# levje/TrackToLearn

Measured on AMD Instinct MI355X. Metric: streamline-steps/s at n_actor=262144, higher is better.
Workload: dtype f32

## Files before the change

### tracktolearn_amd/csrc/ttl_hip.hip

```cpp
#include <hip/hip_runtime.h>

#include <atomic>
#include <chrono>
#include <cmath>
#include <cstdarg>
#include <cstdio>
#include <cstdlib>
#include <cstring>
#include <new>

#include "ttl_hip.h"

#include "ttl_internal.h"

#include <map>
#include <mutex>

namespace {
thread_local char g_err[512] = "";
}

int ttl_detail_fail(int code, const char *fmt, ...) {
    va_list ap;
    va_start(ap, fmt);
// ... 125 lines not shown
    float p1z, float p2x, float p2y, float p2z, int n_pts, float &ux, float &uy,
    float &uz, float &wx, float &wy, float &wz) {
    int bits = 0;
    if (n_pts >= P.max_nb_steps) bits |= TTL_FLAG_LENGTH;
    unit3(p2x - p1x, p2y - p1y, p2z - p1z, ux, uy, uz);
    wx = wy = wz = 0.f;
    if (n_pts >= 3) {
        unit3(p1x - p0x, p1y - p0y, p1z - p0z, wx, wy, wz);
        if (P.curv_enabled) {
            const float dot = (ux * wx + uy * wy) + uz * wz;
            if (dot <= P.curv_dot_max && dot >= -1.0f) bits |= TTL_FLAG_CURVATURE;
        }
    }
    if (outside_mask(P, p2x, p2y, p2z)) bits |= TTL_FLAG_MASK;
    return bits;
}

__device__ __forceinline__ void block_ranks(int *__restrict__ rank_out,
                                            int *__restrict__ counts_out, int i,
                                            bool active, bool keep) {
    const unsigned long long m = __ballot(keep);
    const int lane = threadIdx.x & 63;
    const int wave = threadIdx.x >> 6;
    const int below = __popcll(m & ((1ull << lane) - 1ull));
    __shared__ int wave_total[BLOCK / 64];
    if (lane == 0) wave_total[wave] = __popcll(m);
    __syncthreads();
    int before = 0;
#pragma unroll
    for (int w = 0; w < BLOCK / 64; ++w)
        if (w < wave) before += wave_total[w];
    if (active) rank_out[i] = before + below;
    if (threadIdx.x == 0) {
        int tot = 0;
#pragma unroll
        for (int w = 0; w < BLOCK / 64; ++w) tot += wave_total[w];
        counts_out[blockIdx.x] = tot;
    }
}

__device__ __forceinline__ void block_survivor_ranks(const EnvParams &P, int i,
                                                     bool active, bool keep) {
    block_ranks(P.rank, P.block_counts, i, active, keep);
}

template <int MODE>
__device__ __forceinline__ bool advance_row(
    const EnvParams &P, int g, int i, const float *__restrict__ actions,
    const double *__restrict__ noise, int L, double *__restrict__ reward_out,
    uint8_t *__restrict__ done_out) {
    bool stop = false;
    {
        float *h = P.hist + (size_t)g * (size_t)(P.max_nb_steps + 1) * 3;
        float4 *l2 = reinterpret_cast<float4 *>(P.last2 + 8 * (size_t)g);
        const float4 q0 = l2[0], q1 = l2[1];
        const float p0x = q0.x, p0y = q0.y, p0z = q0.z;
        const float p1x = q1.x, p1y = q1.y, p1z = q1.z;
        const float ax = actions[(size_t)i * 3 + 0];
        const float ay = actions[(size_t)i * 3 + 1];
        const float az = actions[(size_t)i * 3 + 2];

        float p2x, p2y, p2z;
        if (MODE == TTL_MODE_F32) {
            const float s = sqrtf((ax * ax + ay * ay) + az * az);
            float dx = (ax / s) * P.step32;
            float dy = (ay / s) * P.step32;
            float dz = (az / s) * P.step32;
            if (L == 1) {
                const float tx = p1x + dx, ty = p1y + dy, tz = p1z + dz;
                const bool flip = first_step_flips(P, tx, ty, tz);
                dx = flip ? -dx : dx;
                dy = flip ? -dy : dy;
                dz = flip ? -dz : dz;
            }
            p2x = p1x + dx;
            p2y = p1y + dy;
            p2z = p1z + dz;
        } else {
            double dx, dy, dz;
            if (MODE == TTL_MODE_F32NORM) {
                const float s = sqrtf((ax * ax + ay * ay) + az * az);
                dx = (double)(ax / s) * P.step64;
                dy = (double)(ay / s) * P.step64;
                dz = (double)(az / s) * P.step64;
            } else {
                double a0 = (double)ax, a1 = (double)ay, a2 = (double)az;
                if (noise) {
                    a0 = a0 + noise[(size_t)i * 3 + 0];
                    a1 = a1 + noise[(size_t)i * 3 + 1];
                    a2 = a2 + noise[(size_t)i * 3 + 2];
                } else {
                    a0 = a0 + 0.0;
                    a1 = a1 + 0.0;
                    a2 = a2 + 0.0;
                }
                const double s = sqrt((a0 * a0 + a1 * a1) + a2 * a2);
                dx = (a0 / s) * P.step64;
                dy = (a1 / s) * P.step64;
                dz = (a2 / s) * P.step64;
            }
            if (L == 1) {
                const float tx = (float)((double)p1x + dx);
                const float ty = (float)((double)p1y + dy);
                const float tz = (float)((double)p1z + dz);
                const bool flip = first_step_flips(P, tx, ty, tz);
                dx = flip ? -dx : dx;
                dy = flip ? -dy : dy;
                dz = flip ? -dz : dz;
            }
            p2x = (float)((double)p1x + dx);
            p2y = (float)((double)p1y + dy);
            p2z = (float)((double)p1z + dz);
        }
        h[L * 3 + 0] = p2x;
        h[L * 3 + 1] = p2y;
        h[L * 3 + 2] = p2z;
        l2[0] = q1;
        l2[1] = float4{p2x, p2y, p2z, 0.0f};

        const int n_pts = L + 1;
        float ux, uy, uz, wx, wy, wz;
        const int bits = stopping_bits(P, p0x, p0y, p0z, p1x, p1y, p1z, p2x, p2y,
                                       p2z, n_pts, ux, uy, uz, wx, wy, wz);

        stop = bits != 0;
        if (stop) {
            P.flags[g] = bits;
            P.dones[g] = 1;
        }
        done_out[i] = stop ? 1 : 0;

        if (reward_out) {
            double rew = 0.0;
            if (P.compute_reward && P.align_w > 0.0f) {
                int vi = (int)p1x, vj = (int)p1y, vk = (int)p1z;
                vi = min(max(vi, 0), P.peaks_dim[0] - 1);
                vj = min(max(vj, 0), P.peaks_dim[1] - 1);
                vk = min(max(vk, 0), P.peaks_dim[2] - 1);
                const float *pk =
                    P.peaks +
                    (((size_t)vi * P.peaks_dim[1] + vj) * P.peaks_dim[2] + vk) * 15;
                const float u0 = nan_to_num(ux), u1 = nan_to_num(uy),
                            u2 = nan_to_num(uz);
                float best = 0.f;
#pragma unroll
                for (int k = 0; k < 5; ++k) {
                    float vx, vy, vz;
                    unit3(pk[3 * k], pk[3 * k + 1], pk[3 * k + 2], vx, vy, vz);
                    vx = nan_to_num(vx);
                    vy = nan_to_num(vy);
                    vz = nan_to_num(vz);
                    const float d = fabsf((vx * u0 + vy * u1) + vz * u2);
                    if (k == 0)
                        best = d;
                    else if (best == best && (d != d || d > best))
                        best = d;
                }
                float r32 = best;
                if (n_pts >= 3) {
                    const double f = ((double)u0 * (double)nan_to_num(wx) +
                                      (double)u1 * (double)nan_to_num(wy)) +
                                     (double)u2 * (double)nan_to_num(wz);
                    r32 = (float)((double)r32 * f);
                }
                rew = (double)(P.align_w * r32);
            }
            reward_out[i] = rew;
        }
        P.stop[i] = stop ? 1 : 0;
        *reinterpret_cast<float4 *>(P.head + 4 * (size_t)i) =
            float4{p2x, p2y, p2z, __int_as_float(g)};
// ... 387 lines not shown
    if (n_pts >= 2) {
        bits = stopping_bits(P, t[0], t[1], t[2], t[3], t[4], t[5], t[6], t[7],
                             t[8], n_pts, ux, uy, uz, wx, wy, wz);
    } else {
        bits = (n_pts >= P.max_nb_steps) ? TTL_FLAG_LENGTH : 0;
        if (outside_mask(P, t[6], t[7], t[8])) bits |= TTL_FLAG_MASK;
    }
    out[i] = (uint8_t)bits;
}

__global__ __launch_bounds__(BLOCK) void k_finish(EnvParams P,
                                                  const int *__restrict__ idx,
                                                  int n_active, int n_pts) {
    const int i = blockIdx.x * BLOCK + threadIdx.x;
    if (i >= n_active) return;
    if (P.stop[i]) P.lengths[idx[i]] = n_pts;
}

__global__ __launch_bounds__(BLOCK) void k_copy_rows(
    EnvParams P, int n_active, int width, const float *__restrict__ in,
    float *__restrict__ out, long long pitch) {
    constexpr int LPS = 64;
    const int row = blockIdx.x * (BLOCK / LPS) + threadIdx.x / LPS;
    const int sub = threadIdx.x % LPS;
    if (row >= n_active) return;
    const int pos = P.surv_pos[row];
    if (pos < 0) return;
    const float *src = in + (size_t)row * (size_t)pitch;
    float *dst = out + (size_t)pos * (size_t)pitch;
    for (int f = sub; f < width; f += LPS) dst[f] = src[f];
}

__global__ __launch_bounds__(BLOCK) void k_pack_streamlines(
    const float *__restrict__ hist, long long row_pitch, const long long *__restrict__ keep,
    const long long *__restrict__ offsets, int n, float *__restrict__ out) {
    const int i = blockIdx.x * (BLOCK / 64) + (threadIdx.x >> 6);
    if (i >= n) return;
    const int lane = threadIdx.x & 63;
    const int floats = (int)keep[i] * 3;
    const float *src = hist + (size_t)i * (size_t)row_pitch;
    float *dst = out + (size_t)offsets[i] * 3;
    for (int f = lane; f < floats; f += 64) dst[f] = src[f];
}

__global__ __launch_bounds__(BLOCK) void k_reset(EnvParams P, int *idx,
                                                 const float *__restrict__ seeds,
                                                 int n) {
    const int i = blockIdx.x * BLOCK + threadIdx.x;
    if (i >= n) return;
    float *h = P.hist + (size_t)i * (size_t)(P.max_nb_steps + 1) * 3;
    h[0] = seeds[(size_t)i * 3 + 0];
    h[1] = seeds[(size_t)i * 3 + 1];
    h[2] = seeds[(size_t)i * 3 + 2];
    float4 *l2 = reinterpret_cast<float4 *>(P.last2 + 8 * (size_t)i);
    l2[0] = float4{0.0f, 0.0f, 0.0f, 0.0f};
    l2[1] = float4{h[0], h[1], h[2], 0.0f};
    P.flags[i] = 0;
    P.lengths[i] = 1;
    P.dones[i] = 0;
    idx[i] = i;
}

__global__ __launch_bounds__(BLOCK) void k_pack_sh(const float *__restrict__ src,
                                                   float *__restrict__ dst, int X, int Y,
                                                   int Z, int C, int pitch, int brick,
                                                   unsigned sx, unsigned sy) {
    const long long t = (long long)blockIdx.x * BLOCK + threadIdx.x;
    const long long total = (long long)X * Y * Z * pitch;
    if (t >= total) return;
    const long long v = t / pitch;
    const int c = (int)(t - v * pitch);
    const int z = (int)(v % Z), y = (int)((v / Z) % Y), x = (int)(v / ((long long)Z * Y));
    size_t rec;
    if (brick)
        rec = (size_t)(x >> 2) * sx + (size_t)(x & 3) * 16 + (size_t)(y >> 2) * sy +
              (size_t)(y & 3) * 4 + (size_t)(z >> 2) * 64 + (size_t)(z & 3);
    else
        rec = (size_t)v;
    dst[rec * pitch + c] = (c < C) ? src[v * C + c] : 0.0f;
}

__device__ __forceinline__ unsigned mix32(unsigned h) {
    h ^= h >> 16;
    h *= 0x85EBCA6Bu;
    h ^= h >> 13;
    h *= 0xC2B2AE35u;
    h ^= h >> 16;
    return h;
}

__device__ __forceinline__ float scripted_noise(unsigned seed, unsigned step,
                                                unsigned gid, unsigned comp) {
    const unsigned base = mix32(seed * 0x9E3779B1u + step) ^
                          mix32(gid * 0x27D4EB2Fu + comp * 0x165667B1u + 0x1234567u);
    float acc = 0.0f;
#pragma unroll
    for (unsigned k = 0; k < 4; ++k) {
        const unsigned h = mix32(base + k * 0x9E3779B9u);
        acc = acc + (float)(h >> 8) * 5.9604644775390625e-08f;
    }
    return (acc - 2.0f) * 1.7320508075688772f;
}

__global__ __launch_bounds__(BLOCK) void k_scripted_actions(
    const float *__restrict__ state, long long pitch, int dir_offset,
    const int *__restrict__ idx, int n, unsigned seed, unsigned step,
    float wobble, float *__restrict__ actions) {
    const int i = blockIdx.x * BLOCK + threadIdx.x;
    if (i >= n) return;
    const unsigned gid = (unsigned)idx[i];
    const float n0 = scripted_noise(seed, step, gid, 0);
    const float n1 = scripted_noise(seed, step, gid, 1);
    const float n2 = scripted_noise(seed, step, gid, 2);
    float a0 = n0, a1 = n1, a2 = n2;
    if (step > 0) {
        const float *row = state + (size_t)i * (size_t)pitch + dir_offset;
        const float px = row[0], py = row[1], pz = row[2];
        float s = sqrtf((px * px + py * py) + pz * pz);
        if (!(s > 0.0f)) s = 1.0f;
        a0 = px / s + wobble * n0;
        a1 = py / s + wobble * n1;
        a2 = pz / s + wobble * n2;
    }
    actions[(size_t)i * 3 + 0] = a0;
    actions[(size_t)i * 3 + 1] = a1;
    actions[(size_t)i * 3 + 2] = a2;
}

__global__ __launch_bounds__(BLOCK) void k_scripted_actions_fr(
    EnvParams P, const float *__restrict__ state, long long pitch, int dir_offset,
    const int *__restrict__ idx_a, const int *__restrict__ idx_b, int n_rows,
    unsigned seed, float wobble, float *__restrict__ actions) {
    const int *live = P.counts + TTL_FR_LIVE;
    const int n = min(live[0], n_rows);
    const unsigned step = (unsigned)(live[1] - 1);
    const int *idx = live[2] ? idx_b : idx_a;
    const int i = blockIdx.x * BLOCK + threadIdx.x;
    if (i >= n) return;
    const unsigned gid = (unsigned)idx[i];
    const float n0 = scripted_noise(seed, step, gid, 0);
    const float n1 = scripted_noise(seed, step, gid, 1);
    const float n2 = scripted_noise(seed, step, gid, 2);
    float a0 = n0, a1 = n1, a2 = n2;
    if (step > 0) {
        const float *row = state + (size_t)i * (size_t)pitch + dir_offset;
        const float px = row[0], py = row[1], pz = row[2];
        float s = sqrtf((px * px + py * py) + pz * pz);
        if (!(s > 0.0f)) s = 1.0f;
        a0 = px / s + wobble * n0;
        a1 = py / s + wobble * n1;
        a2 = pz / s + wobble * n2;
    }
    actions[(size_t)i * 3 + 0] = a0;
    actions[(size_t)i * 3 + 1] = a1;
    actions[(size_t)i * 3 + 2] = a2;
}

__global__ __launch_bounds__(BLOCK) void k_mask_classes(
    const double *__restrict__ coef, int nx, int ny, int nz, double thr,
    uint8_t *__restrict__ cls) {
    const long long t = (long long)blockIdx.x * BLOCK + threadIdx.x;
    const long long total = (long long)nx * ny * nz;
    if (t >= total) return;
    const int fz = (int)(t % nz), fy = (int)((t / nz) % ny), fx = (int)(t / ((long long)nz * ny));
    double lo = INFINITY, hi = -INFINITY;
    for (int a = 0; a < 4; ++a) {
        const int ia = mirror_fold(fx - 1 + a, nx);
        for (int b = 0; b < 4; ++b) {
            const int ib = mirror_fold(fy - 1 + b, ny);
            const double *line = coef + ((size_t)ia * ny + ib) * nz;
            for (int d = 0; d < 4; ++d) {
                const double v = line[mirror_fold(fz - 1 + d, nz)];
                lo = fmin(lo, v);
                hi = fmax(hi, v);
            }
        }
    }
    const double margin = 1e-9 * (1.0 + fabs(thr) + fmax(fabs(lo), fabs(hi)));
    uint8_t c = 0;
    if (lo >= thr + margin) c = 1;
    else if (hi < thr - margin) c = 2;
    if (!(lo == lo) || !(hi == hi)) c = 0;
    cls[t] = c;
}

inline size_t align_up(size_t v, size_t a) { return (v + a - 1) / a * a; }

}

struct ttl_env {
    ttl_env_desc d;
    EnvParams P;
    int length;
    int n_active;
    int cur;
    int stepped;
    int last_order;
    int last_n;
    uint8_t *last_done;
    int *proc[2];
    char *order_ws;
    size_t order_ws_bytes;
    int proc_cur;
    int use_proc;
    int n_slots;
    int tail_fused;
    int tail_fused_max;
    int state_kernel;
    hipStream_t side;
    hipEvent_t ev_prefix;
    hipEvent_t ev_counts;
    int counts_pending;
    const int32_t *host_counts;
    const int32_t *host_probe;
    int *host_dev;
    int poll_seq;
    hipStream_t poll_stream;
    int fuse_small;
    int poll_counts;
    int local_sort;
    int n_exact;
    int fr_cap;
    int *fr_host_word;
    int prof_on;
    int prof_mask;
    int prof_cap;
    int prof_n[TTL_PROFILE_CLASSES];
    hipEvent_t *prof_ev[TTL_PROFILE_CLASSES];
};

static void log_gather_rows(int n_rows) {
    static FILE *f = []() -> FILE * {
        const char *path = getenv("TTL_GATHER_ROWS_LOG");
        return path && *path ? fopen(path, "a") : nullptr;
    }();
    if (f) {
        fprintf(f, "%d\n", n_rows);
        fflush(f);
    }
}

static void prof_mark(ttl_env *e, int which, int stop, hipStream_t s) {
    if (!e->prof_on || !((e->prof_mask >> which) & 1) ||
        e->prof_n[which] >= e->prof_cap)
        return;
    (void)hipEventRecord(e->prof_ev[which][2 * e->prof_n[which] + stop], s);
    if (stop) e->prof_n[which]++;
}

extern "C" {

const char *ttl_last_error(void) { return g_err; }
uint32_t ttl_abi_version(void) { return TTL_ABI_VERSION; }
size_t ttl_env_desc_size(void) { return sizeof(ttl_env_desc); }

size_t ttl_env_workspace_bytes(int32_t n_max) {
    if (n_max < 0) return 0;
    const size_t n = (size_t)n_max;
    const size_t nb = (n + BLOCK - 1) / BLOCK + 1;
    size_t b = 0;
    b += align_up(n, 256);
    b += 6 * align_up(n * sizeof(int), 256);
    b += 2 * align_up(n * 4 * sizeof(float), 256);
    b += align_up(n * 8 * sizeof(float), 256);
    b += 2 * align_up(n * 2 * sizeof(int), 256);
    b += align_up(n * sizeof(int), 256);
    b += 2 * align_up(nb * sizeof(int), 256);
    b += 256;
    b += ttl_detail_order_workspace_bytes(n);
    return b;
}

int64_t ttl_sh_volume_records(const int32_t *dim, int32_t layout) {
    if (!dim || dim[0] < 1 || dim[1] < 1 || dim[2] < 1) return 0;
    if (layout == TTL_SH_BRICK4)
        return (int64_t)((dim[0] + 3) / 4) * ((dim[1] + 3) / 4) * ((dim[2] + 3) / 4) * 64;
    return (int64_t)dim[0] * dim[1] * dim[2];
}

struct VmmBlock {
    hipMemGenericAllocationHandle_t handle;
    size_t size;
};
static std::mutex g_vmm_mutex;
static std::map<void *, VmmBlock> g_vmm_blocks;

static hipError_t vmm_alloc(int device, size_t bytes, void **out) {
    hipMemAllocationProp prop{};
    prop.type = hipMemAllocationTypePinned;
    prop.location.type = hipMemLocationTypeDevice;
    prop.location.id = device;
    size_t gran = 0;
    hipError_t e = hipMemGetAllocationGranularity(&gran, &prop,
                                                  hipMemAllocationGranularityRecommended);
    if (e != hipSuccess || gran == 0) return e != hipSuccess ? e : hipErrorInvalidValue;
    const size_t size = (bytes + gran - 1) / gran * gran;
    VmmBlock b{};
    b.size = size;
    if ((e = hipMemCreate(&b.handle, size, &prop, 0)) != hipSuccess) return e;
    void *va = nullptr;
    if ((e = hipMemAddressReserve(&va, size, gran, nullptr, 0)) != hipSuccess) {
        (void)hipMemRelease(b.handle);
        return e;
    }
    hipMemAccessDesc acc{};
    acc.location = prop.location;
    acc.flags = hipMemAccessFlagsProtReadWrite;
    if ((e = hipMemMap(va, size, 0, b.handle, 0)) != hipSuccess ||
        (e = hipMemSetAccess(va, size, &acc, 1)) != hipSuccess) {
        (void)hipMemUnmap(va, size);
        (void)hipMemAddressFree(va, size);
        (void)hipMemRelease(b.handle);
        return e;
    }
    std::lock_guard<std::mutex> lock(g_vmm_mutex);
    g_vmm_blocks[va] = b;
    *out = va;
// ... 37 lines not shown

int ttl_volume_free(void *ptr) {
    if (!ptr) return TTL_OK;
    {
        std::unique_lock<std::mutex> lock(g_vmm_mutex);
        auto it = g_vmm_blocks.find(ptr);
        if (it != g_vmm_blocks.end()) {
            const VmmBlock b = it->second;
            g_vmm_blocks.erase(it);
            lock.unlock();
            HIP_TRY(hipDeviceSynchronize());
            HIP_TRY(hipMemUnmap(ptr, b.size));
            HIP_TRY(hipMemAddressFree(ptr, b.size));
            HIP_TRY(hipMemRelease(b.handle));
            return TTL_OK;
        }
    }
    HIP_TRY(hipFree(ptr));
    return TTL_OK;
}

int ttl_pack_sh_volume(const float *src, float *dst, const int32_t *dim, int32_t n_coef,
                       int32_t coef_pitch, int32_t layout, void *hip_stream) {
    if (!src || !dst || !dim || dim[0] < 1 || dim[1] < 1 || dim[2] < 1 || n_coef <= 0 ||
        coef_pitch < n_coef || (coef_pitch & 3) ||
        (layout != TTL_SH_LINEAR && layout != TTL_SH_BRICK4))
        return fail(TTL_ERR_INVALID, "ttl_pack_sh_volume: bad arguments");
    if (((uintptr_t)dst) & 15)
        return fail(TTL_ERR_INVALID, "ttl_pack_sh_volume: dst must be 16B aligned");
    const long long total = (long long)dim[0] * dim[1] * dim[2] * coef_pitch;
    const long long blocks = (total + BLOCK - 1) / BLOCK;
    if (blocks > 0x7fffffffLL)
        return fail(TTL_ERR_INVALID, "ttl_pack_sh_volume: volume too large");
    hipStream_t s = (hipStream_t)hip_stream;
    const int brick = layout == TTL_SH_BRICK4;
    unsigned sx = 0, sy = 0;
    if (brick) {
        HIP_TRY(hipMemsetAsync(dst, 0, (size_t)ttl_sh_volume_records(dim, layout) *
                                           coef_pitch * sizeof(float), s));
        sy = (unsigned)((dim[2] + 3) / 4) * 64u;
        sx = (unsigned)((dim[1] + 3) / 4) * sy;
    }
    hipLaunchKernelGGL(k_pack_sh, dim3((unsigned)blocks), dim3(BLOCK), 0, s, src, dst, dim[0],
                       dim[1], dim[2], n_coef, coef_pitch, brick, sx, sy);
    HIP_TRY(hipGetLastError());
    return TTL_OK;
}

int ttl_mask_classes(const double *mask_coef, const int32_t *dim, double threshold,
                     uint8_t *classes_out, void *hip_stream) {
    if (!mask_coef || !dim || !classes_out || dim[0] < 1 || dim[1] < 1 || dim[2] < 1)
        return fail(TTL_ERR_INVALID, "ttl_mask_classes: bad arguments");
    const long long total = (long long)dim[0] * dim[1] * dim[2];
    hipLaunchKernelGGL(k_mask_classes, dim3((unsigned)((total + BLOCK - 1) / BLOCK)),
                       dim3(BLOCK), 0, (hipStream_t)hip_stream, mask_coef, dim[0],
                       dim[1], dim[2], threshold, classes_out);
    HIP_TRY(hipGetLastError());
    return TTL_OK;
}

int ttl_env_create(const ttl_env_desc *desc, ttl_env **out) {
    if (!desc || !out) return fail(TTL_ERR_INVALID, "ttl_env_create: null argument");
    const ttl_env_desc &d = *desc;
    if (d.abi_version != TTL_ABI_VERSION)
        return fail(TTL_ERR_INVALID, "ttl_env_create: abi_version %u != %u",
                    d.abi_version, TTL_ABI_VERSION);
    if (d.mode != TTL_MODE_F32 && d.mode != TTL_MODE_F64DIR &&
        d.mode != TTL_MODE_F32NORM)
        return fail(TTL_ERR_INVALID, "ttl_env_create: bad mode %d", d.mode);
    for (int a = 0; a < 3; ++a) {
        if (d.sh_dim[a] <= 0 || d.mask_dim[a] <= 0)
            return fail(TTL_ERR_INVALID, "ttl_env_create: non-positive volume dim");
        if (d.compute_reward && d.peaks_dim[a] <= 0)
            return fail(TTL_ERR_INVALID, "ttl_env_create: non-positive peaks dim");
    }
    if (d.sh_layout != TTL_SH_LINEAR && d.sh_layout != TTL_SH_BRICK4)
        return fail(TTL_ERR_INVALID, "ttl_env_create: bad sh_layout %d", d.sh_layout);
    if (d.n_coef <= 0 || d.coef_pitch < d.n_coef || (d.coef_pitch & 3))
        return fail(TTL_ERR_INVALID, "ttl_env_create: coef_pitch must be a multiple of 4 >= n_coef");
    if (!d.sh_packed || (((uintptr_t)d.sh_packed) & 15))
        return fail(TTL_ERR_INVALID, "ttl_env_create: sh_packed null or not 16B aligned");
    if (!d.mask_coef || (((uintptr_t)d.mask_coef) & 7))
        return fail(TTL_ERR_INVALID, "ttl_env_create: mask_coef null or misaligned");
    if (d.compute_reward && !d.peaks)
        return fail(TTL_ERR_INVALID, "ttl_env_create: compute_reward without peaks");
    if (d.n_dirs < 0 || d.max_nb_steps < 1 || d.n_max < 1)
        return fail(TTL_ERR_INVALID, "ttl_env_create: bad n_dirs/max_nb_steps/n_max");
    if (!(d.step_size_vox > 0.0))
        return fail(TTL_ERR_INVALID, "ttl_env_create: step_size_vox must be > 0");
    if (!d.streamlines || !d.flags || !d.lengths || !d.dones || !d.idx_a || !d.idx_b)
        return fail(TTL_ERR_INVALID, "ttl_env_create: null state buffer");
    if (!d.workspace || d.workspace_bytes < ttl_env_workspace_bytes(d.n_max) ||
        (((uintptr_t)d.workspace) & 255))
        return fail(TTL_ERR_INVALID, "ttl_env_create: workspace too small or not 256B aligned");

    ttl_env *e = new (std::nothrow) ttl_env;
    if (!e) return fail(TTL_ERR_INVALID, "ttl_env_create: out of host memory");
    e->d = d;
    EnvParams &P = e->P;
    memset(&P, 0, sizeof(P));
    P.mode = d.mode;
    for (int a = 0; a < 3; ++a) {
        P.sh_dim[a] = d.sh_dim[a];
        P.mask_dim[a] = d.mask_dim[a];
        P.peaks_dim[a] = d.peaks_dim[a];
    }
    P.n_coef = d.n_coef;
    P.coef_pitch = d.coef_pitch;
    P.sh = d.sh_packed;
    P.sh_shift = d.sh_coord_shift;
    P.sh_brick = d.sh_layout == TTL_SH_BRICK4;
    if (P.sh_brick) {
        P.sh_sy = (unsigned)((d.sh_dim[2] + 3) / 4) * 64u;
        P.sh_sx = (unsigned)((d.sh_dim[1] + 3) / 4) * P.sh_sy;
    } else {
        P.sh_sy = (unsigned)d.sh_dim[2];
        P.sh_sx = (unsigned)d.sh_dim[1] * (unsigned)d.sh_dim[2];
    }
    P.mask_coef = d.mask_coef;
    P.mask_cls = d.mask_classes;
    P.mask_thr = d.mask_threshold;
    P.peaks = d.peaks;
    P.compute_reward = d.compute_reward;
    P.align_w = (float)d.alignment_weighting;
    P.n_dirs = d.n_dirs;
    P.max_nb_steps = d.max_nb_steps;
    P.step64 = d.step_size_vox;
    P.step32 = (float)d.step_size_vox;
    P.radius = d.neigh_radius_vox;
    P.curv_enabled = d.curvature_enabled;
    P.curv_dot_max = d.curv_dot_max;
    P.hist = d.streamlines;
    P.flags = d.flags;
    P.lengths = d.lengths;
    P.dones = d.dones;
    const size_t n = (size_t)d.n_max;
    const size_t nb = (n + BLOCK - 1) / BLOCK + 1;
    char *w = (char *)d.workspace;
    P.stop = (uint8_t *)w;        w += align_up(n, 256);
    P.rank = (int *)w;            w += align_up(n * sizeof(int), 256);
    P.surv_pos = (int *)w;        w += align_up(n * sizeof(int), 256);
    P.row_dest = (int *)w;        w += align_up(n * sizeof(int), 256);
    P.block_counts = (int *)w;    w += align_up(nb * sizeof(int), 256);
    P.proc_rank = (int *)w;       w += align_up(n * sizeof(int), 256);
    P.proc_counts = (int *)w;     w += align_up(nb * sizeof(int), 256);
    e->proc[0] = (int *)w;        w += align_up(n * sizeof(int), 256);
    e->proc[1] = (int *)w;        w += align_up(n * sizeof(int), 256);
    P.head = (float *)w;          w += align_up(n * 4 * sizeof(float), 256);
    P.slot_head = (float *)w;     w += align_up(n * 4 * sizeof(float), 256);
    P.last2 = (float *)w;         w += align_up(n * 8 * sizeof(float), 256);
    P.pos_dest = (int *)w;        w += align_up(n * 2 * sizeof(int), 256);
    P.stop_list = (int *)w;       w += align_up(n * 2 * sizeof(int), 256);
    P.slot_dest = (int *)w;       w += align_up(n * sizeof(int), 256);
    P.counts = (int *)w;          w += 256;
    e->order_ws = w;
    e->order_ws_bytes = ttl_detail_order_workspace_bytes(n);
    e->length = 0;
    e->n_active = 0;
    e->cur = 0;
    e->stepped = 0;
    e->last_order = TTL_ORDER_ACTIVE;
    e->last_n = 0;
    e->last_done = nullptr;
    e->proc_cur = 0;
    e->use_proc = 0;
    e->state_kernel = 4;
    if (const char *v = getenv("TTL_STATE_KERNEL")) e->state_kernel = atoi(v);
    P.slot_rec = e->state_kernel != 2;
    P.xcd_remap = 1;
    if (const char *v = getenv("TTL_XCD_REMAP")) P.xcd_remap = atoi(v);
    P.xcd_rot = 0;
    if (const char *v = getenv("TTL_XCD_ROTATE")) P.xcd_rot = atoi(v) & 7;
    P.store_flavour = 0;
    if (const char *v = getenv("TTL_STORE_FLAVOUR")) P.store_flavour = atoi(v);
    e->side = nullptr;
    e->ev_prefix = nullptr;
    e->ev_counts = nullptr;
    e->counts_pending = 0;
    e->host_counts = nullptr;
    e->host_probe = nullptr;
    e->host_dev = nullptr;
    e->poll_seq = 0;
    e->poll_stream = nullptr;
    e->fuse_small = 1;
    if (const char *v = getenv("TTL_FUSE_SMALL")) e->fuse_small = atoi(v);
    P.fuse_max_rows = 64 * BLOCK;
    if (const char *v = getenv("TTL_FUSE_MAX_ROWS")) {
        const int rows = atoi(v);
        P.fuse_max_rows = rows < BLOCK ? BLOCK : rows > TTL_FUSE_MAX_BLOCKS * BLOCK
                                                     ? TTL_FUSE_MAX_BLOCKS * BLOCK : rows;
    }
    e->local_sort = 1;
    P.persist_rows = 0;
    if (const char *v = getenv("TTL_GATHER_PERSIST_ROWS")) P.persist_rows = atoi(v);
    e->tail_fused = 1;
    if (const char *v = getenv("TTL_TAIL_FUSED")) e->tail_fused = atoi(v);
    e->tail_fused_max = 262144;
    if (const char *v = getenv("TTL_TAIL_FUSED_MAX_ROWS")) e->tail_fused_max = atoi(v);
    if (e->tail_fused_max > TTL_TAIL_MAX_BLOCKS * BLOCK) e->tail_fused_max = TTL_TAIL_MAX_BLOCKS * BLOCK;
    e->n_slots = 0;
    if (const char *v = getenv("TTL_LOCAL_SORT")) e->local_sort = atoi(v);
    e->poll_counts = 1;
    if (const char *v = getenv("TTL_POLL_COUNTS")) e->poll_counts = atoi(v);
    e->n_exact = 0;
    e->fr_cap = 0;
    e->fr_host_word = nullptr;
    e->prof_mask = (1 << TTL_PROFILE_CLASSES) - 1;
    e->prof_on = 0;
    e->prof_cap = 0;
    for (int k = 0; k < TTL_PROFILE_CLASSES; ++k) {
        e->prof_n[k] = 0;
        e->prof_ev[k] = nullptr;
    }
    *out = e;
    return TTL_OK;
}

static void prof_free(ttl_env *env) {
    for (int k = 0; k < TTL_PROFILE_CLASSES; ++k) {
        if (env->prof_ev[k]) {
            for (int j = 0; j < 2 * env->prof_cap; ++j) (void)hipEventDestroy(env->prof_ev[k][j]);
            delete[] env->prof_ev[k];
            env->prof_ev[k] = nullptr;
        }
        env->prof_n[k] = 0;
    }
    env->prof_cap = 0;
// ... 548 lines not shown
```

### tracktolearn_amd/csrc/ttl_internal.h

```cpp
#ifndef TTL_INTERNAL_H
#define TTL_INTERNAL_H
#include <hip/hip_runtime.h>

#include <cstdint>

#include "ttl_hip.h"

int ttl_detail_fail(int code, const char *fmt, ...) __attribute__((format(printf, 2, 3)));
#define fail ttl_detail_fail

#define HIP_TRY(expr)                                                        \
    do {                                                                     \
        hipError_t e_ = (expr);                                              \
        if (e_ != hipSuccess)                                                \
            return fail(TTL_ERR_HIP, "%s: %s", #expr, hipGetErrorString(e_)); \
    } while (0)

constexpr int TTL_BLOCK = 256;

struct EnvParams {
    int mode;
    int sh_dim[3];
    int n_coef;
    int coef_pitch;
    const float *sh;
    float sh_shift;
    int sh_brick;
    unsigned sh_sx, sh_sy;
    int mask_dim[3];
    const double *mask_coef;
    const uint8_t *mask_cls;
    double mask_thr;
    int peaks_dim[3];
    const float *peaks;
    int compute_reward;
    float align_w;
    int n_dirs;
    int max_nb_steps;
    double step64;
    float step32;
    float radius;
    int curv_enabled;
    float curv_dot_max;
    float *hist;
    int *flags;
    int *lengths;
    uint8_t *dones;
    uint8_t *stop;
    float *head;
    int *pos_dest;
    float *last2;
    int *rank;
    int *surv_pos;
    int *row_dest;
    int *stop_list;
    int *block_counts;
    int *proc_rank;
    int *proc_counts;
    float *slot_head;
    int *slot_dest;
    int slot_rec;
    int store_flavour;
    int xcd_remap;
    int xcd_rot;
    int *counts;
    int fuse_max_rows;
    int persist_rows;
};

constexpr int TTL_FUSE_MAX_BLOCKS = 256;

constexpr int TTL_FR_LIVE = 8;
constexpr int TTL_FR_SNAP = 16;

__device__ __forceinline__ unsigned vox_x(const EnvParams &P, int x) {
    return P.sh_brick ? (unsigned)(x >> 2) * P.sh_sx + (unsigned)(x & 3) * 16u
                      : (unsigned)x * P.sh_sx;
}
__device__ __forceinline__ unsigned vox_y(const EnvParams &P, int y) {
    return P.sh_brick ? (unsigned)(y >> 2) * P.sh_sy + (unsigned)(y & 3) * 4u
                      : (unsigned)y * P.sh_sy;
}
__device__ __forceinline__ unsigned vox_z(const EnvParams &P, int z) {
    return P.sh_brick ? (unsigned)(z >> 2) * 64u + (unsigned)(z & 3) : (unsigned)z;
}

inline size_t ttl_detail_sh_records(const EnvParams &P) {
    if (!P.sh_brick) return (size_t)P.sh_dim[0] * P.sh_dim[1] * P.sh_dim[2];
    return (size_t)((P.sh_dim[0] + 3) / 4) * ((P.sh_dim[1] + 3) / 4) *
           ((P.sh_dim[2] + 3) / 4) * 64;
}

int ttl_detail_launch_state(const EnvParams &P, int state_kernel, const int *idx,
                            const int *row_dest, const int *proc, int n_rows, int L,
                            float *out, int64_t pitch, hipStream_t s);
bool ttl_detail_state_dedupes(const EnvParams &P, int state_kernel);
bool ttl_detail_can_fuse_tail(const EnvParams &P, int n_active);
int ttl_detail_launch_fused_tail(const EnvParams &P, const int *idx, int *idx_next,
                                 int n_active, int order, int n_pts, float *out,
                                 int64_t pitch, int *host_word, int seq, hipStream_t s);
int ttl_detail_launch_fused_tail_fr(const EnvParams &P, int *idx_a, int *idx_b, int n_cap,
                                    float *out, int64_t pitch, int *host_word,
                                    hipStream_t s);
size_t ttl_detail_order_workspace_bytes(size_t n);
int ttl_detail_refresh_order(const EnvParams &P, const int *idx, int n, char *ws,
                             size_t ws_bytes, int *order_out, hipStream_t s);
#endif
```

### tracktolearn_amd/csrc/ttl_order.hip

```cpp
#include "ttl_internal.h"

#include <cstdlib>
#include <cstring>

#include <rocprim/device/device_radix_sort.hpp>

namespace {
constexpr int BLOCK = TTL_BLOCK;

__global__ __launch_bounds__(BLOCK) void k_order_keys(const float *__restrict__ last2,
                                                      const int *__restrict__ idx, int n,
                                                      int nbx, int nby, int nbz, int fine,
                                                      unsigned *__restrict__ keys,
                                                      int *__restrict__ rows) {
    const int i = blockIdx.x * BLOCK + threadIdx.x;
    if (i >= n) return;
    const float *p = last2 + 8 * (size_t)idx[i] + 4;
    const int nb[3] = {nbx, nby, nbz};
    unsigned b[3], m = 0;
#pragma unroll
    for (int a = 0; a < 3; ++a) {
        const float vox = floorf(p[a] + 0.5f);
        const float v = floorf(vox * 0.125f);
        b[a] = (unsigned)fminf(fmaxf(v == v ? v : 0.0f, 0.0f), (float)(nb[a] - 1));
        const unsigned l = (unsigned)fminf(fmaxf(vox == vox ? vox - 8.0f * v : 0.0f, 0.0f), 7.0f);
        m |= ((l & 1u) << (2 - a)) | ((l & 2u) << (4 - a)) | ((l & 4u) << (6 - a));
    }
    unsigned key;
    if (fine & 2) {
        key = 0;
#pragma unroll
        for (int bit = 0; bit < 10; ++bit)
            key |= (((b[0] >> bit) & 1u) << (3 * bit + 2)) | (((b[1] >> bit) & 1u) << (3 * bit + 1)) |
                   (((b[2] >> bit) & 1u) << (3 * bit));
    } else {
        key = (b[0] * (unsigned)nby + b[1]) * (unsigned)nbz + b[2];
    }
    if (fine & 1) key = (key << 9) | m;
    keys[i] = key;
    rows[i] = i;
}

constexpr int SORT_ITEMS = 8;
constexpr int SORT_CHUNK = BLOCK * SORT_ITEMS;
constexpr int SORT_MAX_BINS = 16384;

__global__ __launch_bounds__(BLOCK) void k_count(const unsigned *__restrict__ keys, int n,
                                                 int bins, unsigned *__restrict__ gcount) {
    extern __shared__ unsigned s_bin[];
    for (int b = threadIdx.x; b < bins; b += BLOCK) s_bin[b] = 0;
    __syncthreads();
    const int base = blockIdx.x * SORT_CHUNK;
#pragma unroll
    for (int k = 0; k < SORT_ITEMS; ++k) {
        const int i = base + k * BLOCK + threadIdx.x;
        if (i < n) atomicAdd(&s_bin[keys[i]], 1u);
    }
    __syncthreads();
    for (int b = threadIdx.x; b < bins; b += BLOCK) {
        const unsigned c = s_bin[b];
        if (c) atomicAdd(&gcount[b], c);
    }
}

__global__ __launch_bounds__(1024) void k_scan(const unsigned *__restrict__ gcount,
                                               unsigned *__restrict__ gcursor, int bins) {
    __shared__ unsigned s_part[1024 / 64];
    const int per = (bins + 1023) / 1024;
    const int lo = threadIdx.x * per;
    unsigned mine = 0;
// ... 117 lines not shown
```

### tracktolearn_amd/csrc/ttl_state.hip

```cpp
#include "ttl_internal.h"

#pragma clang fp contract(fast)

namespace {
constexpr int BLOCK = TTL_BLOCK;

template <int LPS>
__global__ __launch_bounds__(BLOCK) void k_state(
    EnvParams P, const int *__restrict__ idx, const int *__restrict__ row_dest,
    const int *__restrict__ proc, int n_rows, int L, float *__restrict__ out,
    long long pitch) {
    constexpr int GPW = 64 / LPS;
    constexpr int ROWS = (BLOCK / 64) * GPW;
    const int lane = threadIdx.x & 63;
    const int grp = lane / LPS;
    const int slot = blockIdx.x * ROWS + (threadIdx.x >> 6) * GPW + grp;
    const int sub = lane - grp * LPS;
    if (grp >= GPW || slot >= n_rows) return;
    const int row = proc ? proc[slot] : slot;
    if (row < 0) return;
    const int g = idx ? idx[row] : row;
    const int r = row_dest ? row_dest[row] : row;
    const float *h = P.hist + (size_t)g * (size_t)(P.max_nb_steps + 1) * 3;
    const float px = h[(L - 1) * 3 + 0];
// ... 120 lines not shown
        asm volatile("global_store_dwordx4 %0, %1, off sc1" : : "v"(o), "v"(v) : "memory");
    } else if (flavour == 2) {
        asm volatile("global_store_dwordx4 %0, %1, off nt" : : "v"(o), "v"(v) : "memory");
    } else {
        asm volatile("global_store_dwordx4 %0, %1, off sc0 sc1" : : "v"(o), "v"(v) : "memory");
    }
}

template <bool MERGE_TAIL>
__device__ __forceinline__ void put4(int flavour, float *o, f4 a, int c, int C) {
    if (MERGE_TAIL && (flavour & 8)) {
        const int rem = C & 3;
        const bool last = c + 3 >= C;
        v4f v{a.x, a.y, a.z, a.w};
        int back = 0;
        if (rem == 1) {
            const float py = from_prev_lane(a.y), pz = from_prev_lane(a.z), pw = from_prev_lane(a.w);
            if (last) v = v4f{py, pz, pw, a.x};
            back = last ? 3 : 0;
        } else if (rem == 2) {
            const float pz = from_prev_lane(a.z), pw = from_prev_lane(a.w);
            if (last) v = v4f{pz, pw, a.x, a.y};
            back = last ? 2 : 0;
        } else if (rem == 3) {
            const float pw = from_prev_lane(a.w);
            if (last) v = v4f{pw, a.x, a.y, a.z};
            back = last ? 1 : 0;
        }
        store16(o - back, v, flavour & 7);
        return;
    }
    if (MERGE_TAIL) {
        const f4 p{from_prev_lane(a.x), from_prev_lane(a.y), from_prev_lane(a.z),
                   from_prev_lane(a.w)};
        const int back = (c + 3 < C) ? 0 : 4 - (C - c);
        v4f v{a.x, a.y, a.z, a.w};
        if (back == 1) v = v4f{p.w, a.x, a.y, a.z};
        if (back == 2) v = v4f{p.z, p.w, a.x, a.y};
        if (back == 3) v = v4f{p.y, p.z, p.w, a.x};
        store16(o - back, v, flavour);
        return;
    }
    if (c + 3 < C) {
        store16(o, v4f{a.x, a.y, a.z, a.w}, flavour);
    } else {
        if (c + 0 < C) o[0] = a.x;
        if (c + 1 < C) o[1] = a.y;
        if (c + 2 < C) o[2] = a.z;
    }
}

template <int LPS, bool LOOP, bool MERGE_TAIL>
__device__ __forceinline__ void state_row_dd(const EnvParams &P, float px, float py,
                                             float pz, const float *__restrict__ h, int L,
                                             int sub, float *__restrict__ orow) {
    const int n_seg = L - 1;
    float dvx = 0.0f, dvy = 0.0f, dvz = 0.0f;
    if (sub < P.n_dirs && sub < n_seg) {
        const float *a = h + (L - 2 - sub) * 3;
        const float ax = a[0], ay = a[1], az = a[2];
        const float bx = a[3], by = a[4], bz = a[5];
        dvx = bx - ax;
        dvy = by - ay;
        dvz = bz - az;
    }
    const int C = P.n_coef;
    const int C4 = P.coef_pitch >> 2;
    const int X = P.sh_dim[0], Y = P.sh_dim[1], Z = P.sh_dim[2];
    const char *vol = reinterpret_cast<const char *>(P.sh);
    const float rad = P.radius;

    float cxp = px + rad, cxm = px + (-rad);
    float cyp = py + rad, cym = py + (-rad);
    float czp = pz + rad, czm = pz + (-rad);
    if (P.sh_shift != 0.0f) {
        px += P.sh_shift; py += P.sh_shift; pz += P.sh_shift;
        cxp += P.sh_shift; cxm += P.sh_shift;
        cyp += P.sh_shift; cym += P.sh_shift;
        czp += P.sh_shift; czm += P.sh_shift;
    }
    const float fx = floorf(px), fy = floorf(py), fz = floorf(pz);
    const float dx = px - fx, dy = py - fy, dz = pz - fz;
    const float ex = 1.0f - dx, ey = 1.0f - dy, ez = 1.0f - dz;
    const float fxp = floorf(cxp), fxm = floorf(cxm);
    const float fyp = floorf(cyp), fym = floorf(cym);
    const float fzp = floorf(czp), fzm = floorf(czm);
    const float dxp = cxp - fxp, dxm = cxm - fxm;
    const float dyp = cyp - fyp, dym = cym - fym;
    const float dzp = czp - fzp, dzm = czm - fzm;
    const bool xup = fxp > fx, xdn = fxm < fx;
    const bool yup = fyp > fy, ydn = fym < fy;
    const bool zup = fzp > fz, zdn = fzm < fz;
    const int ix = (int)fminf(fmaxf(fx, -4.0f), (float)X + 4.0f);
    const int iy = (int)fminf(fmaxf(fy, -4.0f), (float)Y + 4.0f);
    const int iz = (int)fminf(fmaxf(fz, -4.0f), (float)Z + 4.0f);
    const unsigned rec = (unsigned)C4 * 16u;
    const unsigned x0 = vox_x(P, clipi(ix - 1, X)) * rec, x1 = vox_x(P, clipi(ix, X)) * rec,
                   x2 = vox_x(P, clipi(ix + 1, X)) * rec, x3 = vox_x(P, clipi(ix + 2, X)) * rec;
    const unsigned y0 = vox_y(P, clipi(iy - 1, Y)) * rec, y1 = vox_y(P, clipi(iy, Y)) * rec,
                   y2 = vox_y(P, clipi(iy + 1, Y)) * rec, y3 = vox_y(P, clipi(iy + 2, Y)) * rec;
    const unsigned z0 = vox_z(P, clipi(iz - 1, Z)) * rec, z1 = vox_z(P, clipi(iz, Z)) * rec,
                   z2 = vox_z(P, clipi(iz + 1, Z)) * rec, z3 = vox_z(P, clipi(iz + 2, Z)) * rec;
#define TTL_VOX(xo, yo, zo) ((xo) + (yo) + (zo))
    for (int c4 = sub; c4 < C4; c4 += LPS) {
        const unsigned cb = (unsigned)c4 * 16u;
        const f4 v000 = ld4(vol, TTL_VOX(x1, y1, z1) + cb), v001 = ld4(vol, TTL_VOX(x1, y1, z2) + cb);
        const f4 v010 = ld4(vol, TTL_VOX(x1, y2, z1) + cb), v011 = ld4(vol, TTL_VOX(x1, y2, z2) + cb);
        const f4 v100 = ld4(vol, TTL_VOX(x2, y1, z1) + cb), v101 = ld4(vol, TTL_VOX(x2, y1, z2) + cb);
        const f4 v110 = ld4(vol, TTL_VOX(x2, y2, z1) + cb), v111 = ld4(vol, TTL_VOX(x2, y2, z2) + cb);
        const f4 zero{0.f, 0.f, 0.f, 0.f};
        const int c = c4 * 4;
        {
// ... 74 lines not shown
    long long pitch, int n_vblocks) {
    constexpr int GPW = 64 / LPS;
    constexpr int ROWS = (BLOCK / 64) * GPW;
    const int lane = threadIdx.x & 63;
    const int grp = lane / LPS;
    const int sub = lane - grp * LPS;
    if (grp >= GPW) return;
    for (int vb = blockIdx.x; vb < n_vblocks; vb += gridDim.x) {
        int blk = vb;
        if (proc && P.xcd_remap) {
            const int nwg = n_vblocks, q = nwg >> 3, rr = nwg & 7, xcd = blk & 7;
            if (P.xcd_rot == 0) {
                blk = (xcd < rr ? xcd * (q + 1) : rr * (q + 1) + (xcd - rr) * q) + (blk >> 3);
            } else {
                const int mine = (xcd + P.xcd_rot) & 7;
                int start = 0;
                for (int r = 0; r < mine; ++r)
                    start += q + ((((r - P.xcd_rot) & 7) < rr) ? 1 : 0);
                blk = start + (blk >> 3);
            }
        }
        const int slot = blk * ROWS + (threadIdx.x >> 6) * GPW + grp;
        if (slot >= n_rows) continue;
        int row, g, r;
        float px, py, pz;
        const bool slot_records = proc && idx && P.slot_rec;
        if (slot_records) {
            const float4 hp = *reinterpret_cast<const float4 *>(P.slot_head + 4 * (size_t)slot);
            px = hp.x;
            py = hp.y;
            pz = hp.z;
            g = __float_as_int(hp.w);
            r = P.slot_dest[slot];
            row = 0;
            if (r < 0) continue;
        } else {
            row = proc ? proc[slot] : slot;
            if (row < 0) continue;
            g = idx ? idx[row] : row;
            r = row_dest ? row_dest[row] : row;
        }
        const float *h = P.hist + (size_t)g * (size_t)(P.max_nb_steps + 1) * 3;
        if (slot_records) {
        } else if (idx) {
            const float4 hp = *reinterpret_cast<const float4 *>(P.head + 4 * (size_t)row);
            px = hp.x;
            py = hp.y;
            pz = hp.z;
        } else {
            px = h[(L - 1) * 3 + 0];
            py = h[(L - 1) * 3 + 1];
            pz = h[(L - 1) * 3 + 2];
        }
        state_row_dd<LPS, LOOP, MERGE_TAIL>(P, px, py, pz, h, L, sub,
                                            out + (size_t)r * (size_t)pitch);
    }
}

template <int LPS, bool MERGE_TAIL, bool FR>
__device__ __forceinline__ void prefix_state_body(
    const EnvParams &P, const int *__restrict__ idx, int *__restrict__ idx_next, int n_active,
    int n_blocks, int order, int n_pts, float *__restrict__ out, long long pitch,
    int *__restrict__ host_word, int seq, int cur) {
    constexpr int GPW = 64 / LPS;
    constexpr int ROWS = (BLOCK / 64) * GPW;
    __shared__ int s_before[TTL_FUSE_MAX_BLOCKS + 1];
    const int lane = threadIdx.x & 63;
    if (threadIdx.x < 64) {
        int c[4];
#pragma unroll
        for (int k = 0; k < 4; ++k)
            c[k] = 4 * lane + k < n_blocks ? P.block_counts[4 * lane + k] : 0;
        const int local = (c[0] + c[1]) + (c[2] + c[3]);
        int v = local;
#pragma unroll
        for (int off = 1; off < 64; off <<= 1) {
            const int t = __shfl_up(v, off);
            if (lane >= off) v += t;
        }
        int run = v - local;
#pragma unroll
        for (int k = 0; k < 4; ++k) {
            s_before[4 * lane + k] = run;
            run += c[k];
        }
        if (lane == 63) s_before[TTL_FUSE_MAX_BLOCKS] = v;
    }
    __syncthreads();
    const int total = s_before[TTL_FUSE_MAX_BLOCKS];
    if (blockIdx.x == 0 && threadIdx.x == 0) {
        P.counts[0] = total;
        P.counts[1] = n_active - total;
        if (FR) {
            int *live = P.counts + TTL_FR_LIVE;
            live[0] = total;
            live[1] = n_active > 0 ? n_pts : n_pts - 1;
            live[2] = n_active > 0 ? cur ^ 1 : cur;
            live[3] = seq;
        }
        if (host_word) {
            __hip_atomic_store(host_word + 0, total, __ATOMIC_RELAXED, __HIP_MEMORY_SCOPE_SYSTEM);
            __hip_atomic_store(host_word + 1, n_active - total, __ATOMIC_RELAXED,
                               __HIP_MEMORY_SCOPE_SYSTEM);
            __hip_atomic_store(host_word + 2, seq, __ATOMIC_RELEASE, __HIP_MEMORY_SCOPE_SYSTEM);
        }
    }
    const int grp = lane / LPS;
    const int row = blockIdx.x * ROWS + (threadIdx.x >> 6) * GPW + grp;
    const int sub = lane - grp * LPS;
    if (grp >= GPW || row >= n_active) return;
    const float4 hp = *reinterpret_cast<const float4 *>(P.head + 4 * (size_t)row);
    const int g = __float_as_int(hp.w);
    const bool stop = P.stop[row] != 0;
    const int pos = s_before[row >> 8] + P.rank[row];
    int dest = row;
    if (order == TTL_ORDER_PARTITION) dest = stop ? total + (row - pos) : pos;
    if (sub == 0) {
        if (!stop) idx_next[pos] = g;
        if (stop && order == TTL_ORDER_PARTITION) P.lengths[g] = n_pts;
        P.surv_pos[row] = stop ? -1 : pos;
        P.row_dest[row] = dest;
        if (stop)
            *reinterpret_cast<int2 *>(P.stop_list + 2 * (size_t)(row - pos)) = int2{row, g};
    }
    const float *h = P.hist + (size_t)g * (size_t)(P.max_nb_steps + 1) * 3;
    state_row_dd<LPS, false, MERGE_TAIL>(P, hp.x, hp.y, hp.z, h, n_pts, sub,
                                         out + (size_t)dest * (size_t)pitch);
}

template <int LPS, bool MERGE_TAIL>
__global__ __launch_bounds__(BLOCK, 4) void k_prefix_state(
    EnvParams P, const int *__restrict__ idx, int *__restrict__ idx_next, int n_active,
    int n_blocks, int order, int n_pts, float *__restrict__ out, long long pitch,
    int *__restrict__ host_word, int seq) {
    prefix_state_body<LPS, MERGE_TAIL, false>(P, idx, idx_next, n_active, n_blocks, order,
                                              n_pts, out, pitch, host_word, seq, 0);
}

template <int LPS, bool MERGE_TAIL>
__global__ __launch_bounds__(BLOCK, 4) void k_prefix_state_fr(
    EnvParams P, int *__restrict__ idx_a, int *__restrict__ idx_b, int n_blocks,
    float *__restrict__ out, long long pitch, int *__restrict__ host_word) {
    const int *snap = P.counts + TTL_FR_SNAP;
    const int n_active = snap[0], L = snap[1], cur = snap[2], seq = snap[3] + 1;
    if (snap[4]) {
        if (blockIdx.x == 0 && threadIdx.x == 0) {
            P.counts[TTL_FR_LIVE + 3] = seq;
            if (host_word)
                __hip_atomic_store(host_word + 2, seq, __ATOMIC_RELEASE, __HIP_MEMORY_SCOPE_SYSTEM);
        }
        return;
    }
    prefix_state_body<LPS, MERGE_TAIL, true>(P, cur ? idx_b : idx_a, cur ? idx_a : idx_b,
                                             n_active, n_blocks, TTL_ORDER_PARTITION, L + 1,
                                             out, pitch, host_word, seq, cur);
}

}

bool ttl_detail_can_fuse_tail(const EnvParams &P, int n_active) {
    const int C4 = P.coef_pitch >> 2;
    const size_t vol_bytes = ttl_detail_sh_records(P) * P.coef_pitch * sizeof(float);
    return n_active <= P.fuse_max_rows && P.radius > 0.0f && P.radius < 1.0f &&
           vol_bytes < (1ull << 32) && C4 <= 16 && P.n_coef >= 4;
}

int ttl_detail_launch_fused_tail(const EnvParams &P, const int *idx, int *idx_next,
                                 int n_active, int order, int n_pts, float *out,
                                 int64_t pitch, int *host_word, int seq, hipStream_t s) {
    const int C4 = P.coef_pitch >> 2;
    const int n_blocks = (n_active + BLOCK - 1) / BLOCK;
#define TTL_LAUNCH_FUSED(LPS)                                                        \
    do {                                                                             \
        const int rows_per_block = (BLOCK / 64) * (64 / LPS);                        \
        const dim3 grid((n_active + rows_per_block - 1) / rows_per_block);           \
        hipLaunchKernelGGL((k_prefix_state<LPS, true>), grid, dim3(BLOCK), 0, s, P, idx, \
                           idx_next, n_active, n_blocks, order, n_pts, out,          \
                           (long long)pitch, host_word, seq);                        \
    } while (0)
// ... 75 lines not shown
```

Before: 808.2 million.

## Keep a five-point per-streamline ring to serve direction reads; add Bezier hull mask classing

The per-streamline last-two-points cache grows into a 16-float ring holding the last five points. When n_dirs is small enough, the state kernel reads previous-direction segments from this contiguous ring instead of from the strided history buffer. The intent is to cut scattered history reads in the state build, at the cost of extra ring reads and writes on every step. The mask-class kernel also gains a Bezier convex-hull refinement that tightens the classification of ambiguous voxels; this is a one-time preprocessing accuracy change.

```diff
diff --git a/tracktolearn_amd/csrc/ttl_hip.hip b/tracktolearn_amd/csrc/ttl_hip.hip
--- a/tracktolearn_amd/csrc/ttl_hip.hip
+++ b/tracktolearn_amd/csrc/ttl_hip.hip
@@ -201,10 +201,10 @@
     bool stop = false;
     {
         float *h = P.hist + (size_t)g * (size_t)(P.max_nb_steps + 1) * 3;
-        float4 *l2 = reinterpret_cast<float4 *>(P.last2 + 8 * (size_t)g);
-        const float4 q0 = l2[0], q1 = l2[1];
-        const float p0x = q0.x, p0y = q0.y, p0z = q0.z;
-        const float p1x = q1.x, p1y = q1.y, p1z = q1.z;
+        float4 *ring = reinterpret_cast<float4 *>(P.last2 + TTL_RING_FLOATS * (size_t)g);
+        const float4 q0 = ring[0], q1 = ring[1], q2 = ring[2], q3 = ring[3];
+        const float p0x = q2.y, p0y = q2.z, p0z = q2.w;
+        const float p1x = q3.x, p1y = q3.y, p1z = q3.z;
         const float ax = actions[(size_t)i * 3 + 0];
         const float ay = actions[(size_t)i * 3 + 1];
         const float az = actions[(size_t)i * 3 + 2];
@@ -264,8 +264,10 @@
         h[L * 3 + 0] = p2x;
         h[L * 3 + 1] = p2y;
         h[L * 3 + 2] = p2z;
-        l2[0] = q1;
-        l2[1] = float4{p2x, p2y, p2z, 0.0f};
+        ring[0] = float4{q0.w, q1.x, q1.y, q1.z};
+        ring[1] = float4{q1.w, q2.x, q2.y, q2.z};
+        ring[2] = float4{q2.w, q3.x, q3.y, q3.z};
+        ring[3] = float4{p2x, p2y, p2z, 0.0f};
 
         const int n_pts = L + 1;
         float ux, uy, uz, wx, wy, wz;
@@ -759,9 +761,12 @@
     h[0] = seeds[(size_t)i * 3 + 0];
     h[1] = seeds[(size_t)i * 3 + 1];
     h[2] = seeds[(size_t)i * 3 + 2];
-    float4 *l2 = reinterpret_cast<float4 *>(P.last2 + 8 * (size_t)i);
-    l2[0] = float4{0.0f, 0.0f, 0.0f, 0.0f};
-    l2[1] = float4{h[0], h[1], h[2], 0.0f};
+    float4 *ring = reinterpret_cast<float4 *>(P.last2 + TTL_RING_FLOATS * (size_t)i);
+    const float4 zero{0.0f, 0.0f, 0.0f, 0.0f};
+    ring[0] = zero;
+    ring[1] = zero;
+    ring[2] = zero;
+    ring[3] = float4{h[0], h[1], h[2], 0.0f};
     P.flags[i] = 0;
     P.lengths[i] = 1;
     P.dones[i] = 0;
@@ -863,6 +868,18 @@
     actions[(size_t)i * 3 + 2] = a2;
 }
 
+__device__ __forceinline__ void bezier_axis(double &c0, double &c1, double &c2, double &c3) {
+    const double b0 = (c0 + 4.0 * c1 + c2) / 6.0;
+    const double b1 = (2.0 * c1 + c2) / 3.0;
+    const double b2 = (c1 + 2.0 * c2) / 3.0;
+    const double b3 = (c1 + 4.0 * c2 + c3) / 6.0;
+    c0 = b0;
+    c1 = b1;
+    c2 = b2;
+    c3 = b3;
+}
+
+template <bool HULL>
 __global__ __launch_bounds__(BLOCK) void k_mask_classes(
     const double *__restrict__ coef, int nx, int ny, int nz, double thr,
     uint8_t *__restrict__ cls) {
@@ -870,16 +887,20 @@
     const long long total = (long long)nx * ny * nz;
     if (t >= total) return;
     const int fz = (int)(t % nz), fy = (int)((t / nz) % ny), fx = (int)(t / ((long long)nz * ny));
+    double v[4][4][4];
     double lo = INFINITY, hi = -INFINITY;
+#pragma unroll
     for (int a = 0; a < 4; ++a) {
         const int ia = mirror_fold(fx - 1 + a, nx);
+#pragma unroll
         for (int b = 0; b < 4; ++b) {
             const int ib = mirror_fold(fy - 1 + b, ny);
             const double *line = coef + ((size_t)ia * ny + ib) * nz;
+#pragma unroll
             for (int d = 0; d < 4; ++d) {
-                const double v = line[mirror_fold(fz - 1 + d, nz)];
-                lo = fmin(lo, v);
-                hi = fmax(hi, v);
+                v[a][b][d] = line[mirror_fold(fz - 1 + d, nz)];
+                lo = fmin(lo, v[a][b][d]);
+                hi = fmax(hi, v[a][b][d]);
             }
         }
     }
@@ -888,6 +909,37 @@
     if (lo >= thr + margin) c = 1;
     else if (hi < thr - margin) c = 2;
     if (!(lo == lo) || !(hi == hi)) c = 0;
+    if (HULL && c == 0) {
+#pragma unroll
+        for (int a = 0; a < 4; ++a)
+#pragma unroll
+            for (int b = 0; b < 4; ++b) bezier_axis(v[a][b][0], v[a][b][1], v[a][b][2], v[a][b][3]);
+#pragma unroll
+        for (int a = 0; a < 4; ++a)
+#pragma unroll
+            for (int d = 0; d < 4; ++d) bezier_axis(v[a][0][d], v[a][1][d], v[a][2][d], v[a][3][d]);
+#pragma unroll
+        for (int b = 0; b < 4; ++b)
+#pragma unroll
+            for (int d = 0; d < 4; ++d) bezier_axis(v[0][b][d], v[1][b][d], v[2][b][d], v[3][b][d]);
+        double blo = INFINITY, bhi = -INFINITY;
+        bool finite = true;
+#pragma unroll
+        for (int a = 0; a < 4; ++a)
+#pragma unroll
+            for (int b = 0; b < 4; ++b)
+#pragma unroll
+                for (int d = 0; d < 4; ++d) {
+                    const double w = v[a][b][d];
+                    blo = fmin(blo, w);
+                    bhi = fmax(bhi, w);
+                    finite = finite && fabs(w) <= 1.79769313486231570e308;
+                }
+        if (finite) {
+            if (blo >= thr + margin) c = 1;
+            else if (bhi < thr - margin) c = 2;
+        }
+    }
     cls[t] = c;
 }
 
@@ -969,7 +1021,7 @@
     b += align_up(n, 256);
     b += 6 * align_up(n * sizeof(int), 256);
     b += 2 * align_up(n * 4 * sizeof(float), 256);
-    b += align_up(n * 8 * sizeof(float), 256);
+    b += align_up(n * TTL_RING_FLOATS * sizeof(float), 256);
     b += 2 * align_up(n * 2 * sizeof(int), 256);
     b += align_up(n * sizeof(int), 256);
     b += 2 * align_up(nb * sizeof(int), 256);
@@ -1113,9 +1165,15 @@
     if (!mask_coef || !dim || !classes_out || dim[0] < 1 || dim[1] < 1 || dim[2] < 1)
         return fail(TTL_ERR_INVALID, "ttl_mask_classes: bad arguments");
     const long long total = (long long)dim[0] * dim[1] * dim[2];
-    hipLaunchKernelGGL(k_mask_classes, dim3((unsigned)((total + BLOCK - 1) / BLOCK)),
-                       dim3(BLOCK), 0, (hipStream_t)hip_stream, mask_coef, dim[0],
-                       dim[1], dim[2], threshold, classes_out);
+    const char *bounds = getenv("TTL_MASK_CLASS_BOUNDS");
+    const bool hull = !(bounds && strcmp(bounds, "taps") == 0);
+    const dim3 grid((unsigned)((total + BLOCK - 1) / BLOCK));
+    if (hull)
+        hipLaunchKernelGGL(k_mask_classes<true>, grid, dim3(BLOCK), 0, (hipStream_t)hip_stream,
+                           mask_coef, dim[0], dim[1], dim[2], threshold, classes_out);
+    else
+        hipLaunchKernelGGL(k_mask_classes<false>, grid, dim3(BLOCK), 0, (hipStream_t)hip_stream,
+                           mask_coef, dim[0], dim[1], dim[2], threshold, classes_out);
     HIP_TRY(hipGetLastError());
     return TTL_OK;
 }
@@ -1209,7 +1267,7 @@
     e->proc[1] = (int *)w;        w += align_up(n * sizeof(int), 256);
     P.head = (float *)w;          w += align_up(n * 4 * sizeof(float), 256);
     P.slot_head = (float *)w;     w += align_up(n * 4 * sizeof(float), 256);
-    P.last2 = (float *)w;         w += align_up(n * 8 * sizeof(float), 256);
+    P.last2 = (float *)w;         w += align_up(n * TTL_RING_FLOATS * sizeof(float), 256);
     P.pos_dest = (int *)w;        w += align_up(n * 2 * sizeof(int), 256);
     P.stop_list = (int *)w;       w += align_up(n * 2 * sizeof(int), 256);
     P.slot_dest = (int *)w;       w += align_up(n * sizeof(int), 256);
@@ -1234,6 +1292,8 @@
     if (const char *v = getenv("TTL_XCD_ROTATE")) P.xcd_rot = atoi(v) & 7;
     P.store_flavour = 0;
     if (const char *v = getenv("TTL_STORE_FLAVOUR")) P.store_flavour = atoi(v);
+    P.dir_ring = d.n_dirs < TTL_RING_POINTS;
+    if (const char *v = getenv("TTL_DIR_RING")) P.dir_ring = P.dir_ring && atoi(v) != 0;
     e->side = nullptr;
     e->ev_prefix = nullptr;
     e->ev_counts = nullptr;
diff --git a/tracktolearn_amd/csrc/ttl_internal.h b/tracktolearn_amd/csrc/ttl_internal.h
--- a/tracktolearn_amd/csrc/ttl_internal.h
+++ b/tracktolearn_amd/csrc/ttl_internal.h
@@ -50,6 +50,7 @@
     float *head;
     int *pos_dest;
     float *last2;
+    int dir_ring;
     int *rank;
     int *surv_pos;
     int *row_dest;
@@ -69,6 +70,10 @@
 };
 
 constexpr int TTL_FUSE_MAX_BLOCKS = 256;
+
+constexpr int TTL_RING_FLOATS = 16;
+constexpr int TTL_RING_POINTS = 5;
+constexpr int TTL_RING_NEWEST = 3 * (TTL_RING_POINTS - 1);
 
 constexpr int TTL_FR_LIVE = 8;
 constexpr int TTL_FR_SNAP = 16;
diff --git a/tracktolearn_amd/csrc/ttl_order.hip b/tracktolearn_amd/csrc/ttl_order.hip
--- a/tracktolearn_amd/csrc/ttl_order.hip
+++ b/tracktolearn_amd/csrc/ttl_order.hip
@@ -15,7 +15,7 @@
                                                       int *__restrict__ rows) {
     const int i = blockIdx.x * BLOCK + threadIdx.x;
     if (i >= n) return;
-    const float *p = last2 + 8 * (size_t)idx[i] + 4;
+    const float *p = last2 + TTL_RING_FLOATS * (size_t)idx[i] + TTL_RING_NEWEST;
     const int nb[3] = {nbx, nby, nbz};
     unsigned b[3], m = 0;
 #pragma unroll
diff --git a/tracktolearn_amd/csrc/ttl_state.hip b/tracktolearn_amd/csrc/ttl_state.hip
--- a/tracktolearn_amd/csrc/ttl_state.hip
+++ b/tracktolearn_amd/csrc/ttl_state.hip
@@ -196,12 +196,13 @@
 
 template <int LPS, bool LOOP, bool MERGE_TAIL>
 __device__ __forceinline__ void state_row_dd(const EnvParams &P, float px, float py,
-                                             float pz, const float *__restrict__ h, int L,
-                                             int sub, float *__restrict__ orow) {
+                                             float pz, int g, const float *__restrict__ h,
+                                             int L, int sub, float *__restrict__ orow) {
     const int n_seg = L - 1;
     float dvx = 0.0f, dvy = 0.0f, dvz = 0.0f;
     if (sub < P.n_dirs && sub < n_seg) {
-        const float *a = h + (L - 2 - sub) * 3;
+        const float *a = P.dir_ring ? P.last2 + TTL_RING_FLOATS * (size_t)g + (TTL_RING_NEWEST - 3) - 3 * sub
+                                    : h + (L - 2 - sub) * 3;
         const float ax = a[0], ay = a[1], az = a[2];
         const float bx = a[3], by = a[4], bz = a[5];
         dvx = bx - ax;
@@ -382,7 +383,7 @@
             py = h[(L - 1) * 3 + 1];
             pz = h[(L - 1) * 3 + 2];
         }
-        state_row_dd<LPS, LOOP, MERGE_TAIL>(P, px, py, pz, h, L, sub,
+        state_row_dd<LPS, LOOP, MERGE_TAIL>(P, px, py, pz, g, h, L, sub,
                                             out + (size_t)r * (size_t)pitch);
     }
 }
@@ -454,7 +455,7 @@
             *reinterpret_cast<int2 *>(P.stop_list + 2 * (size_t)(row - pos)) = int2{row, g};
     }
     const float *h = P.hist + (size_t)g * (size_t)(P.max_nb_steps + 1) * 3;
-    state_row_dd<LPS, false, MERGE_TAIL>(P, hp.x, hp.y, hp.z, h, n_pts, sub,
+    state_row_dd<LPS, false, MERGE_TAIL>(P, hp.x, hp.y, hp.z, g, h, n_pts, sub,
                                          out + (size_t)dest * (size_t)pitch);
 }
 
```

Result: slower. 800.1 million (-1.0%).
